# deepqmc/deepqmc

Measured on NVIDIA H100. Metric: walker.local-energies/sec, higher is better.
Workload: dtype f32

## Files before the change

deepqmc_b200/csrc/engine.cu:

```cuda
#include <algorithm>
#include <array>
#include <cstdio>
#include <cstdlib>
#include <cstring>
#include <limits>
#include <map>
#include <mutex>
#include <optional>
#include <string>
#include <type_traits>
#include <vector>

#include "dqmc_b200.h"
#include "kernels_mcmc.cuh"
#include "kernels_slater.cuh"
#include "kernels_trunk.cuh"
#include "kernels_gnn.cuh"
#include "kernels_bwd.cuh"
#include "attn_mma.cuh"
#if !defined(DQMC_NO_TCGEN05)
#include "gemm_wgmma.cuh"
#include "fused_tc.cuh"
#include "trunk_tc.cuh"
#endif

namespace dq {

struct ParamEntry {
  std::string name;
  int64_t offset;
  int rows, cols;
};

static inline size_t align_up(size_t x, size_t a = 256) { return (x + a - 1) / a * a; }

template <class W>
static double last_above(W w, double lo, double eps) {
  double hi = lo > 0.0 ? 2 * lo : 1.0;
  while (w(hi) >= eps) { lo = hi; hi *= 2; }
  for (;;) {
    const double mid = lo + 0.5 * (hi - lo);
    if (mid <= lo || mid >= hi) break;
    (w(mid) >= eps ? lo : hi) = mid;
  }
  return lo;
}

template <class T>
static double ecp_cutoff_rc2(const T* nl, int L, int Tn, bool on) {
  const double inf = std::numeric_limits<double>::infinity(), eps = std::ldexp(1.0, -100);
  if (!on) return inf;
  for (int l = 0; l < L; ++l)
    for (int t = 0; t < Tn; ++t)
      if ((double)nl[(l * 2 + 1) * Tn + t] != 0.0 && !((double)nl[(l * 2) * Tn + t] > 0.0)) return inf;
  auto w = [&](double d2) {
    double s = 0.0;
    for (int l = 0; l < L; ++l)
      for (int t = 0; t < Tn; ++t)
        s += (2 * l + 1) * std::fabs((double)nl[(l * 2 + 1) * Tn + t]) * std::exp(-(double)nl[(l * 2) * Tn + t] * d2);
    return s;
  };
  if (w(0.0) < eps) return -inf;
  return last_above(w, 0.0, eps);
}

template <class T>
static double ecp_force_cutoff_rc2(const T* nl, int L, int Tn, bool on) {
  const double rc2 = ecp_cutoff_rc2(nl, L, Tn, on), eps = std::ldexp(1.0, -100);
  if (rc2 == std::numeric_limits<double>::infinity()) return rc2;
  double peak = 0.0;
  for (int l = 0; l < L; ++l)
    for (int t = 0; t < Tn; ++t)
      if ((double)nl[(l * 2 + 1) * Tn + t] != 0.0) peak = std::max(peak, 0.5 / (double)nl[(l * 2) * Tn + t]);
  auto wd = [&](double d2) {
    double s = 0.0;
    for (int l = 0; l < L; ++l)
      for (int t = 0; t < Tn; ++t) {
        const double a = (double)nl[(l * 2) * Tn + t];
        s += (2 * l + 1) * 2 * a * std::fabs((double)nl[(l * 2 + 1) * Tn + t]) * std::sqrt(d2) * std::exp(-a * d2);
      }
    return s;
  };
  return std::max(rc2, wd(peak) >= eps ? last_above(wd, peak, eps) : peak);
}

struct Switches {
  bool tc_trunk = true;
  bool tc_f16 = true;
  std::optional<bool> attn_fl_mma;
  std::optional<int> attn_tb, attn_nt;
  bool attn_generic = false;
  bool no_fuse_tanh = false;
  bool slater_generic = false;
  bool slater_fwd1 = false;
  bool ecp_cutoff = true;
  bool ecp_env_table = true;
  bool ecp_emb_table = true;
  int nsms = 0;
  bool trunk_phases = false;
};

inline Switches read_switches() {
  auto env = [](const char* name) { return std::getenv(name); };
  auto num = [&](const char* name) { const char* ev = env(name); return ev ? std::optional<int>(std::atoi(ev)) : std::nullopt; };
  Switches s;
  s.tc_trunk = num("DQMC_TC_TRUNK").value_or(1) != 0;
  s.tc_f16 = num("DQMC_TC_F16").value_or(1) != 0;
  if (auto v = num("DQMC_ATTN_FL_MMA")) s.attn_fl_mma = *v != 0;
  s.attn_tb = num("DQMC_ATTN_TB");
  s.attn_nt = num("DQMC_ATTN_NT");
  s.attn_generic = env("DQMC_ATTN_GENERIC");
  s.no_fuse_tanh = env("DQMC_NO_FUSE_TANH");
  s.slater_generic = env("DQMC_SLATER_GENERIC");
  s.slater_fwd1 = env("DQMC_SLATER_FWD1");
  s.ecp_cutoff = num("DQMC_ECP_CUTOFF").value_or(1) != 0;
  s.ecp_env_table = !env("DQMC_ECP_ENV_TABLE_OFF");
  s.ecp_emb_table = !env("DQMC_ECP_EMB_TABLE_OFF");
  s.nsms = num("DQMC_NSMS").value_or(0);
  s.trunk_phases = num("DQMC_TRUNK_PHASES").value_or(0) != 0;
  return s;
}

struct EngineBase {
  dqmc_config cfg;
  int device = 0;
  std::string err;
  int64_t launches = 0;
  int64_t ecp_forwards = 0;
  std::vector<ParamEntry> entries;
  int64_t total = 0;
  bool dry = false;
  bool plan_only = false;
  mutable const char* dry_hwm = nullptr;
  void note_hwm(const void* q) const { if (dry && (const char*)q > dry_hwm) dry_hwm = (const char*)q; }
  mutable std::vector<unsigned char*> emu_guards;
  bool prof = false;
  double prof_flops = 0;
  int64_t prof_n = 0;
  double prof_cls_flops[3] = {0, 0, 0};
  int64_t prof_cls_n[3] = {0, 0, 0};
  std::vector<int> prof_cls;
#ifndef DQMC_EMU
  std::vector<cudaEvent_t> prof_ev;
  void prof_note(cudaEvent_t e0, cudaEvent_t e1, double flops, int cls) {
    prof_ev.push_back(e0); prof_ev.push_back(e1);
    prof_cls.push_back(cls);
    prof_flops += flops; prof_cls_flops[cls] += flops;
    ++prof_n; ++prof_cls_n[cls];
  }
#endif
  virtual ~EngineBase() {}
  virtual int set_params(const double* host, int64_t n, cudaStream_t st) = 0;
  virtual int64_t ws_bytes(int B, int mode) = 0;
  virtual int64_t ws_bytes_min(int B, int mode) = 0;
  virtual int debug_plan(int B, int mode, int64_t wsb, int64_t* planned, int64_t* carved) = 0;
  virtual int stats_pack(const void* E, const void* stats, int B, double* out, cudaStream_t st) = 0;
  virtual int debug_mlp_block(int layer, const void* O, const void* X, void* Out, int rows, cudaStream_t st) = 0;
  virtual int debug_trunk(const void* X0, void* Out, int rows, cudaStream_t st) = 0;
  virtual int debug_attention(int layer, const void* QKV, void* O, int rows, int S, int32_t* kernel, cudaStream_t st) = 0;
  virtual int debug_mlp(int layer, int S, const void* O, const void* X, void* Out, void* scratch, int rows, int32_t* path,
                        cudaStream_t st) = 0;
  virtual int debug_trunk_phases(uint64_t* out, int n) = 0;
  virtual int debug_slater(const void* r, const void* R, const void* BF, int rows, int S, void* dsign, void* dlog, void* dgrad,
                           void* dlap, int32_t* kernel, cudaStream_t st) = 0;
  virtual int debug_det_sum(const void* r, const void* R, const void* dsign, const void* dlog, const void* dgrad,
                            const void* dlap, int B, int S, void* sign, void* logp, void* grad, void* stats,
                            cudaStream_t st) = 0;
  virtual int forward(const void* r, const void* R, int Rb, int B, void* sign, void* logp, void* ws, int64_t wsb,
                      cudaStream_t st) = 0;
  virtual int local_energy(const void* r, const void* R, int Rb, int B, uint64_t seed, const void* twist, void* E,
                           void* stats, void* sign, void* logp, void* grad, void* ws, int64_t wsb,
                           cudaStream_t st) = 0;
  virtual int langevin(void* r, void* sign, void* logp, void* force, int32_t* age, void* tau, const void* R, int Rb, int B,
                       int n_sub, double target, int max_age, uint64_t seed, uint64_t step0, uint64_t woff, const void* nn,
                       const void* nu, void* stats, void* ws, int64_t wsb, cudaStream_t st) = 0;
  virtual int vjp_params(const void* r, const void* R, int Rb, int B, const void* weights, void* sign, void* logp,
                         void* grad_params, void* ws, int64_t wsb, cudaStream_t st) = 0;
  virtual int spin(const void* r, const void* R, int Rb, int B, const void* sign, const void* logp, int down_idx, void* s2,
                   void* ratio, void* ws, int64_t wsb, cudaStream_t st) = 0;
  virtual int grad_positions(const void* r, const void* R, int Rb, int B, void* sign, void* logp, void* grad_r, void* grad_R,
                             void* ws, int64_t wsb, cudaStream_t st) = 0;
  virtual int force_terms(const void* r, const void* R, int Rb, int B, const void* grad_r, void* bare, void* zvq, void* Q,
                          cudaStream_t st) = 0;
  virtual int ecp_force(const void* r, const void* R, int Rb, int B, uint64_t seed, const void* twist, void* bare, void* nl,
                        void* ws, int64_t wsb, cudaStream_t st) = 0;
  virtual int orbitals(const void* r, const void* R, int Rb, int B, void* out, void* ws, int64_t wsb, cudaStream_t st) = 0;
  virtual int set_ph(int n_tab, int n_grid, double r_max, const double* tables, const int32_t* tab_of_nuc) = 0;
  virtual int debug_gemm(const char* wname, const char* bname, const void* A, const void* Res, void* C, int Mr, int S,
                         int sliced, int backend, cudaStream_t st) = 0;
  virtual int mcmc(void* r, void* sign, void* logp, int32_t* age, void* tau, const void* R, int Rb, int B, int n_sub,
// ... 397 lines not shown
      std::vector<int> nuc;
      for (int m = 0; m < M; ++m) {
        bool any = false;
        for (int l = 0; l < L; ++l)
          for (int ab = 0; ab < 2; ++ab)
            for (int t = 0; t < Tn; ++t) {
              double v = cfg.ecp_nl[m][l][ab][t];
              np[(((size_t)m * L + l) * 2 + ab) * Tn + t] = (T)v;
              any = any || v != 0.0;
            }
        if (any) nuc.push_back(m);
      }
      J = (int)nuc.size();
      if (J > 0) {
        DQ_CHECK(cudaMalloc((void**)&d_nl_params, sizeof(T) * np.size()));
        DQ_CHECK(cudaMemcpy(d_nl_params, np.data(), sizeof(T) * np.size(), cudaMemcpyHostToDevice));
        DQ_CHECK(cudaMalloc((void**)&d_nl_nuc, sizeof(int) * J));
        DQ_CHECK(cudaMemcpy(d_nl_nuc, nuc.data(), sizeof(int) * J, cudaMemcpyHostToDevice));
        std::vector<double> rc2(J), rc2f(J);
        for (int j = 0; j < J; ++j) {
          rc2[j] = ecp_cutoff_rc2(np.data() + (size_t)nuc[j] * L * 2 * Tn, L, Tn, sw.ecp_cutoff);
          rc2f[j] = ecp_force_cutoff_rc2(np.data() + (size_t)nuc[j] * L * 2 * Tn, L, Tn, sw.ecp_cutoff);
        }
        DQ_CHECK(cudaMalloc((void**)&d_nl_rc2, sizeof(double) * J));
        DQ_CHECK(cudaMemcpy(d_nl_rc2, rc2.data(), sizeof(double) * J, cudaMemcpyHostToDevice));
        DQ_CHECK(cudaMalloc((void**)&d_nl_rc2f, sizeof(double) * J));
        DQ_CHECK(cudaMemcpy(d_nl_rc2f, rc2f.data(), sizeof(double) * J, cudaMemcpyHostToDevice));
      }
    }
#ifndef DQMC_EMU
    {
      int v = 0;
      DQ_CHECK(cudaDeviceGetAttribute(&v, cudaDevAttrMultiProcessorCount, device));
      if (v > 0) n_sms = v;
    }
#endif
    if (sw.nsms >= 1) n_sms = sw.nsms;
    const bool psif = cfg.kind == DQMC_PSIFORMER || trans;
    attn_f32 = psif && !trans && std::is_same<T, float>::value && dh % 16 == 0 && !sw.attn_generic;
    if (sw.attn_tb && *sw.attn_tb >= 1 && *sw.attn_tb <= T3) attn_tb = *sw.attn_tb;
    else attn_tb = attn_f32 ? attn_f32_pick_tb(N, dh, T3, 32 * 1024) : attn_pick_tb<T>(N, dh, T3, 100 * 1024, Mn);
    size_t s_attn = !psif ? 0 : attn_f32 ? attn_f32_smem_bytes(N, dh, attn_tb) : attn_smem_bytes<T>(N, dh, attn_tb, Mn);
    if (!sw.attn_nt) attn_fl_threads = s_attn > 110 * 1024 ? 512 : (s_attn > 56 * 1024 ? 256 : 128);
    else if (*sw.attn_nt >= 32 && *sw.attn_nt <= 1024 && *sw.attn_nt % 32 == 0) attn_fl_threads = *sw.attn_nt;
    attn_fl_mma = attn_f32 && N <= 32 && dh % 16 == 0 && sw.attn_fl_mma.value_or(N >= 20);
    if (attn_fl_mma && !sw.attn_tb) {
      attn_tb = attn_f32_pick_tb(N, dh, T3, 110 * 1024);
      s_attn = attn_f32_smem_bytes(N, dh, attn_tb);
    }
    attn_gen_mma = psif && !attn_f32 && std::is_same<T, float>::value && dh % 16 == 0 &&
                   sw.attn_fl_mma.value_or(N >= 20 && !sw.attn_generic);
    if (attn_gen_mma) {
      if (!sw.attn_tb) attn_tb = attn_pick_tb<T>(N, dh, T3, 110 * 1024, Mn, 4);
      s_attn = attn_smem_bytes<T>(N, dh, attn_tb, Mn, 4);
    }
    size_t s_sl = slater_smem_bytes<T>(N);
    max_smem = s_attn > s_sl ? s_attn : s_sl;
    if (max_smem > 227 * 1024) { err = "system too large for the shared-memory tiling (N)"; return 2; }
    if (attn_f32) {
      if (launch_attn_f32(nullptr, nullptr, 0, 0, 0, 0.f, 0, (int)s_attn, nullptr, true)) return 1;
    } else if (psif) {
      DQ_CHECK(raise_dyn_smem(attn_fl_kernel<T>, (int)s_attn));
      if constexpr (std::is_same<T, float>::value) DQ_CHECK(raise_dyn_smem((attn_fl_kernel<T, true>), (int)s_attn));
    }
    DQ_CHECK(raise_dyn_smem(slater_kernel<T>, (int)s_sl));
    slater_fwd2_ok = N <= 32 && slater_fwd2_smem_bytes<T>(N, M, K) <= 110 * 1024 && !sw.slater_generic && !sw.slater_fwd1;
    if (slater_fwd2_ok) {
      DQ_CHECK(raise_dyn_smem(slater_fwd2_kernel<T, 14>, (int)slater_fwd2_smem_bytes<T>(N, M, K)));
      DQ_CHECK(raise_dyn_smem(slater_fwd2_kernel<T, 16>, (int)slater_fwd2_smem_bytes<T>(N, M, K)));
      DQ_CHECK(raise_dyn_smem(slater_fwd2_kernel<T, 28>, (int)slater_fwd2_smem_bytes<T>(N, M, K)));
      DQ_CHECK(raise_dyn_smem(slater_fwd2_kernel<T, 30>, (int)slater_fwd2_smem_bytes<T>(N, M, K)));
      DQ_CHECK(raise_dyn_smem(slater_fwd2_kernel<T, 32>, (int)slater_fwd2_smem_bytes<T>(N, M, K)));
    }
    attn_mma_ok = psif && std::is_same<T, float>::value && dh == 64 && N + Mn <= 48 && d % 4 == 0 && !sw.attn_generic;
    embed_fwd_ok = psif && d % 4 == 0 && embed_fwd_smem_bytes<T>(M, d) <= 200 * 1024;
    if (embed_fwd_ok)
      DQ_CHECK(raise_dyn_smem(embed_fwd_kernel<T>, (int)embed_fwd_smem_bytes<T>(M, d)));
    if (cfg.gemm_backend == DQMC_GEMM_TCGEN05) {
#if !defined(DQMC_NO_TCGEN05)
      if (!std::is_same<T, float>::value) { err = "DQMC_GEMM_TCGEN05 needs dtype DQMC_F32"; return 2; }
      if (d % 32 != 0) { err = "DQMC_GEMM_TCGEN05 needs embedding_dim % 32 == 0"; return 2; }
      DQ_CHECK(raise_dyn_smem(tc::gemm3x_kernel<false>, tc::SmemLayout::total()));
      DQ_CHECK(raise_dyn_smem(tc::gemm3x_kernel<true>, tc::SmemLayout::total()));
      DQ_CHECK(raise_dyn_smem(tc::mlp_block_f16_kernel<128>, tc::MlpSmem::total()));
      DQ_CHECK(raise_dyn_smem(tc::mlp_block_f16_kernel<256>, tc::MlpSmem::total()));
      DQ_CHECK(raise_dyn_smem(tc::trunk_f16_kernel<1>, tc::TrSmem::total()));
      DQ_CHECK(raise_dyn_smem(tc::trunk_f16_kernel<2>, tc::TrSmem::total()));
      DQ_CHECK(raise_dyn_smem(tc::trunk_f16_kernel<4>, tc::TrSmem::total()));
      DQ_CHECK(raise_dyn_smem(tc::trunk_f16_kernel<8>, tc::TrSmem::total()));
      DQ_CHECK(raise_dyn_smem(tc::trunk_f16_kernel<16>, tc::TrSmem::total()));
      DQ_CHECK(raise_dyn_smem(tc::trunk_f16_kernel<32>, tc::TrSmem::total()));
      if (psif && !trans && d == 256 && H == 4 && N <= 32 && cfg.n_layers <= tc::kTrMaxLayers) {
        DQ_CHECK(cudaMalloc((void**)&d_trunk_maps, sizeof(CUtensorMap) * 8 * cfg.n_layers));
        DQ_CHECK(cudaMalloc((void**)&d_trunk_scratch, (size_t)n_sms * tc::kTrScratchPerCta));
        if (sw.trunk_phases) {
          DQ_CHECK(cudaMalloc((void**)&d_trunk_phase, sizeof(unsigned long long) * tc::kPhases));
          DQ_CHECK(cudaMemset(d_trunk_phase, 0, sizeof(unsigned long long) * tc::kPhases));
        }
      }
#else
      err = "this build has no tensor-core backend"; return 2;
#endif
    }
    return 0;
  }
  ~Engine() override {
    if (plan_only) return;
    cudaFree(d_params); cudaFree(d_params_t); cudaFree(d_stage); cudaFree(d_znuc); cudaFree(d_zval); cudaFree(d_ecp_mask);
    if (d_ecp_loc) cudaFree(d_ecp_loc);
    if (d_nl_params) cudaFree(d_nl_params);
    if (d_nl_nuc) cudaFree(d_nl_nuc);
    if (d_nl_rc2) cudaFree(d_nl_rc2);
    if (d_nl_rc2f) cudaFree(d_nl_rc2f);
    if (d_ph_tabs) cudaFree(d_ph_tabs);
    if (d_ph_nuc) cudaFree(d_ph_nuc);
#if !defined(DQMC_NO_TCGEN05)
    for (auto& kv : tcw) {
      if (kv.second.hi) cudaFree(kv.second.hi);
      if (kv.second.lo) cudaFree(kv.second.lo);
      if (kv.second.h16) cudaFree(kv.second.h16);
    }
    if (d_trunk_maps) cudaFree(d_trunk_maps);
    if (d_trunk_scratch) cudaFree(d_trunk_scratch);
    if (d_trunk_phase) cudaFree(d_trunk_phase);
#endif
  }
  const T* P(const std::string& n) const { return d_params + off(n); }

  int set_ph(int n_tab, int n_grid, double r_max, const double* tables, const int32_t* tab_of_nuc) override {
    if (J > 0 || cfg.ecp_loc_terms > 0) { err = "pseudo-Hamiltonian and Gaussian-type ECP are mutually exclusive"; return 2; }
    if (n_tab < 1 || n_grid < 2 || !(r_max > 0) || !tables || !tab_of_nuc) { err = "bad pseudo-Hamiltonian tables"; return 2; }
    for (int m = 0; m < M; ++m)
      if (tab_of_nuc[m] >= n_tab) { err = "pseudo-Hamiltonian table index out of range"; return 2; }
    std::vector<T> h((size_t)n_tab * 2 * n_grid);
    for (size_t i = 0; i < h.size(); ++i) h[i] = (T)tables[i];
    if (d_ph_tabs) cudaFree(d_ph_tabs);
    if (d_ph_nuc) cudaFree(d_ph_nuc);
    DQ_CHECK(cudaMalloc((void**)&d_ph_tabs, sizeof(T) * h.size()));
    DQ_CHECK(cudaMemcpy(d_ph_tabs, h.data(), sizeof(T) * h.size(), cudaMemcpyHostToDevice));
    DQ_CHECK(cudaMalloc((void**)&d_ph_nuc, sizeof(int) * M));
    DQ_CHECK(cudaMemcpy(d_ph_nuc, tab_of_nuc, sizeof(int) * M, cudaMemcpyHostToDevice));
    ph_G = n_grid; ph_rmax = r_max; ph_on = true;
    return 0;
  }
  PhArgs<T> ph_args(const T* QA) const {
    PhArgs<T> a;
    a.QA = QA; a.tabs = d_ph_tabs; a.tab_of_nuc = d_ph_nuc; a.G = ph_G; a.rmax = (T)ph_rmax;
    return a;
  }

  int set_params(const double* host, int64_t n, cudaStream_t st) override {
    if (n != total) { err = "parameter count mismatch"; return 2; }
    DQ_CHECK(cudaMemcpyAsync(d_stage, host, sizeof(double) * n, cudaMemcpyHostToDevice, st));
    DQ_LAUNCH(convert_kernel<T>, dim3((unsigned)((n + 255) / 256)), dim3(256), 0, st, (const double*)d_stage, d_params, n);
    for (auto& e : entries)
      if (e.rows >= 1 && e.cols >= 1)
        DQ_LAUNCH(transpose_kernel<T>, dim3((e.rows * e.cols + 255) / 256), dim3(256), 0, st, (const T*)(d_params + e.offset),
                  e.rows, e.cols, d_params_t + e.offset);
#if !defined(DQMC_NO_TCGEN05)
    if (use_tc()) {
      std::map<std::string, double> wmax;
      auto group = [](const std::string& n) {
        const size_t k = n.size();
        return (k > 3 && (n.compare(k - 3, 3, ".up") == 0 || n.compare(k - 3, 3, ".dn") == 0)) ? n.substr(0, k - 3) : n;
      };
      for (auto& e : entries) {
// ... 215 lines not shown
    if (B < 1) B = 1;
    const int S = T3 + 2;
    switch (mode) {
      case DQMC_MODE_VJP: return vjp_chunk_bytes(1);
      case DQMC_MODE_GRAD_POS: return has_pos_pass() ? vjp_chunk_bytes(1, true) : 0;
      case DQMC_MODE_MCMC: return sweep_bytes(B, false, 1);
      case DQMC_MODE_LANGEVIN: return sweep_bytes(B, true, 1);
      case DQMC_MODE_LOCAL_ENERGY: return std::max<int64_t>(chunk_bytes(1, S), J > 0 ? ecp_bytes(1, 1) : 0);
      case DQMC_MODE_ECP_FORCE: return J > 0 && has_nl_force() ? ecp_force_bytes(1, 1) : 0;
      case DQMC_MODE_SPIN: {
        const int64_t P = (int64_t)cfg.n_up * cfg.n_down;
        return P ? spin_bytes(1, P, 1) : 0;
      }
      default: return chunk_bytes(1, 1);
    }
  }
  int debug_plan(int B, int mode, int64_t wsb, int64_t* planned, int64_t* carved) override {
    const int64_t pl = ws_bytes(B, mode);
    if (planned) *planned = pl;
    if (wsb <= 0) wsb = pl;
    DryPass dp(this);
    void* ws = plan_base();
    int rc = 0;
    switch (mode) {
      case DQMC_MODE_FORWARD: rc = forward(nullptr, nullptr, 0, B, nullptr, nullptr, ws, wsb, nullptr); break;
      case DQMC_MODE_LOCAL_ENERGY:
        rc = local_energy(nullptr, nullptr, 0, B, 0, nullptr, nullptr, nullptr, nullptr, nullptr, nullptr, ws, wsb, nullptr);
        break;
      case DQMC_MODE_VJP: rc = vjp_params(nullptr, nullptr, 0, B, nullptr, nullptr, nullptr, nullptr, ws, wsb, nullptr); break;
      case DQMC_MODE_MCMC:
        rc = mcmc(nullptr, nullptr, nullptr, nullptr, nullptr, nullptr, 0, B, 1, 0.5, -1, 0, 0, 0, nullptr, nullptr, nullptr, ws, wsb,
                  nullptr, 0.0, nullptr, nullptr);
        break;
      case DQMC_MODE_LANGEVIN:
        rc = langevin(nullptr, nullptr, nullptr, nullptr, nullptr, nullptr, nullptr, 0, B, 1, 0.5, -1, 0, 0, 0, nullptr, nullptr,
                      nullptr, ws, wsb, nullptr);
        break;
      case DQMC_MODE_SPIN: rc = spin(nullptr, nullptr, 0, B, nullptr, nullptr, -1, nullptr, nullptr, ws, wsb, nullptr); break;
      case DQMC_MODE_GRAD_POS:
        rc = grad_positions(nullptr, nullptr, 0, B, nullptr, nullptr, nullptr, nullptr, ws, wsb, nullptr);
        break;
      case DQMC_MODE_ECP_FORCE:
        rc = ecp_force(nullptr, nullptr, 0, B, 0, nullptr, nullptr, has_nl_force() ? ws : nullptr, ws, wsb, nullptr);
        break;
      default: err = "unknown mode"; rc = 2;
    }
    if (carved) *carved = dp.bytes();
    return rc;
  }

  bool can_fuse_act(int S) const {
    if (!use_tc() || sw.no_fuse_tanh) return false;
    if (S == 1) return true;
    return S <= 128 && (128 / S) * S >= 112;
  }
  bool gemm_on_tc(const char* w0, const char* w1, int lda, int ldc, int Kc, const T* bias1) const {
#if !defined(DQMC_NO_TCGEN05)
    return use_tc() && !bias1 && Kc % 32 == 0 && lda % 4 == 0 && ldc % 4 == 0 && tcw.count(w0) && (!w1 || tcw.count(w1));
#else
    return false;
#endif
  }
  int gemm(const T* A, int lda, const char* w0, const char* w1, int zsplit, int ldw, const T* bias, const T* Res,
           int ldr, T* C, int ldc, int Mr, int Nc, int Kc, int S, int sliced, int Nel, cudaStream_t st, int act = 0,
           const T* bias1 = nullptr) {
    if (dry) return 0;
    const T* W0 = P(w0);
    const T* W1 = w1 ? P(w1) : nullptr;
#if !defined(DQMC_NO_TCGEN05)
    if constexpr (std::is_same<T, float>::value) {
      if (gemm_on_tc(w0, w1, lda, ldc, Kc, bias1)) {
        const TcWeight& t0 = tcw.at(w0);
        const TcWeight& t1 = w1 ? tcw.at(w1) : t0;
        tc::Params p;
        p.A = A; p.lda = lda; p.bias = bias; p.Res = Res; p.ldr = ldr; p.C = C; p.ldc = ldc; p.M = Mr; p.N = Nc;
        p.K = Kc; p.S = S; p.sliced = sliced; p.Nel = Nel; p.z_split = zsplit; p.err_flag = nullptr;
        p.act = act;
        p.rpt = (act && S > 1) ? (128 / S) * S : tc::kBM;
        p.a_scale = 1.f; p.unscale = 1.f;
        const bool f16 = S == 1 && sw.tc_f16 && Kc % 64 == 0 && t0.f16 && t1.f16 && t0.wscale == t1.wscale;
        if (f16) { p.a_scale = kActScale; p.unscale = 1.f / (kActScale * t0.wscale); }
        const int MT = (Mr + p.rpt - 1) / p.rpt, NT = (Nc + tc::kBN - 1) / tc::kBN;
        const int n_tiles = (sliced ? Nel : 1) * MT * NT;
#ifndef DQMC_EMU
        cudaEvent_t e0 = nullptr, e1 = nullptr;
        if (prof) { cudaEventCreate(&e0); cudaEventCreate(&e1); cudaEventRecord(e0, st); }
#endif
        if (f16)
          DQ_LAUNCH(tc::gemm3x_kernel<true>, dim3(n_tiles), dim3(tc::kThreads), tc::SmemLayout::total(), st, t0.m16h, t0.m16l,
                    t1.m16h, t1.m16l, p);
        else
          DQ_LAUNCH(tc::gemm3x_kernel<false>, dim3(n_tiles), dim3(tc::kThreads), tc::SmemLayout::total(), st, t0.mh, t0.ml,
                    t1.mh, t1.ml, p);
#ifndef DQMC_EMU
        if (prof) {
          cudaEventRecord(e1, st);
          prof_note(e0, e1, 2.0 * (double)Mr * (sliced ? Nel : 1) * (double)Nc * (double)Kc, 0);
        }
#endif
        return 0;
      }
    }
#endif
    if (act) { err = "internal: fused activation requested on the CUDA-core GEMM"; return 5; }
    GemmArgs<T> g;
    g.A = A; g.lda = lda; g.W0 = W0; g.W1 = W1; g.z_split = zsplit; g.ldw = ldw; g.bias = bias; g.Res = Res;
    g.ldr = ldr; g.C = C; g.ldc = ldc; g.M = Mr; g.N = Nc; g.K = Kc; g.S = S; g.sliced = sliced; g.Nel = Nel;
    g.bias1 = bias1;
    constexpr int BM = 64, BN = 64, BK = 16, TM = 4, TN = 4;
    dim3 grid((Nc + BN - 1) / BN, (Mr + BM - 1) / BM, sliced ? Nel : 1);
#ifndef DQMC_EMU
    cudaEvent_t e0 = nullptr, e1 = nullptr;
    if (prof) { cudaEventCreate(&e0); cudaEventCreate(&e1); cudaEventRecord(e0, st); }
#endif
    DQ_LAUNCH((gemm_kernel<T, BM, BN, BK, TM, TN>), grid, dim3(256), 0, st, g);
#ifndef DQMC_EMU
    if (prof) {
      cudaEventRecord(e1, st);
      prof_note(e0, e1, 2.0 * (double)Mr * (sliced ? Nel : 1) * (double)Nc * (double)Kc, 0);
    }
#endif
    return 0;
  }

  bool can_fuse_mlp(int S, const std::string& pfx) const {
#if !defined(DQMC_NO_TCGEN05)
    if (S != 1 || !use_tc() || !sw.tc_f16 || (d != 128 && d != 256)) return false;
    for (const char* n : {"wo", "w1", "w2"}) {
      auto it = tcw.find(pfx + n);
      if (it == tcw.end() || !it->second.f16_all) return false;
    }
    return true;
#else
    return false;
#endif
  }
  int mlp_block(const std::string& pfx, const T* O, const T* X, T* Out, int rows, cudaStream_t st) {
    if (dry) return 0;
#if !defined(DQMC_NO_TCGEN05)
    if constexpr (std::is_same<T, float>::value) {
      const TcWeight& wo = tcw.at(pfx + "wo");
      const TcWeight& w1 = tcw.at(pfx + "w1");
      const TcWeight& w2 = tcw.at(pfx + "w2");
      tc::MlpParams p;
      p.O = O; p.ldo = d; p.X = X; p.ldx = d; p.Out = Out; p.ldout = d; p.b1 = P(pfx + "b1"); p.b2 = P(pfx + "b2");
      p.M = rows; p.d = d; p.a_scale = kActScale;
      p.us0 = 1.f / (kActScale * wo.wscale); p.us1 = 1.f / (kActScale * w1.wscale); p.us2 = 1.f / (kActScale * w2.wscale);
      p.err_flag = nullptr;
      const int MT = (rows + 127) / 128;
      const int grid = MT < n_sms ? MT : n_sms;
#ifndef DQMC_EMU
      cudaEvent_t e0 = nullptr, e1 = nullptr;
      if (prof) { cudaEventCreate(&e0); cudaEventCreate(&e1); cudaEventRecord(e0, st); }
#endif
      if (d == 256)
        DQ_LAUNCH(tc::mlp_block_f16_kernel<256>, dim3(grid), dim3(tc::kMlpThreads), tc::MlpSmem::total(), st, wo.m16h_all,
                  wo.m16l_all, w1.m16h_all, w1.m16l_all, w2.m16h_all, w2.m16l_all, p);
      else
        DQ_LAUNCH(tc::mlp_block_f16_kernel<128>, dim3(grid), dim3(tc::kMlpThreads), tc::MlpSmem::total(), st, wo.m16h_all,
                  wo.m16l_all, w1.m16h_all, w1.m16l_all, w2.m16h_all, w2.m16l_all, p);
#ifndef DQMC_EMU
      if (prof) {
        cudaEventRecord(e1, st);
        prof_note(e0, e1, 3 * 2.0 * (double)rows * (double)d * (double)d, 1);
      }
#endif
      return 0;
    }
#endif
    err = "internal: fused MLP block without the tensor-core backend";
    return 5;
  }

  int debug_mlp_block(int layer, const void* O, const void* X, void* Out, int rows, cudaStream_t st) override {
    const std::string pfx = "L" + std::to_string(layer) + ".";
    if (!can_fuse_mlp(1, pfx)) { err = "fused MLP block not available for this configuration"; return 2; }
// ... 1785 lines not shown
```

deepqmc_b200/csrc/gemm_wgmma.cuh:

```cuda
#pragma once
#include <cstdint>

#include "tc_ptx.cuh"

namespace dq {
namespace tc {

constexpr int kBM = 128;
constexpr int kBN = 128;
constexpr int kBK = 32;
constexpr int kThreads = 256;

struct Params {
  const float* A; int lda;
  const float* bias;
  const float* Res; int ldr;
  float* C; int ldc;
  int M, N, K;
  int S;
  int sliced, Nel, z_split;
  int act;
  int rpt;
  int* err_flag;
  float a_scale;
// ... 141 lines not shown
  }
  __syncthreads();

  constexpr int P = SmemLayout::kPitch;
  float* st = (float*)smem;
  {
    const int lane = tid & 31;
    const int fr = 64 * wg + 16 * ((tid >> 5) & 3) + (lane >> 2), fc = 2 * (lane & 3);
    const float us = F16 ? p.unscale : 1.f;
#pragma unroll
    for (int j = 0; j < kBN / 8; ++j)
#pragma unroll
      for (int h = 0; h < 2; ++h)
        *(float2*)(st + (fr + 8 * h) * P + 8 * j + fc) = make_float2(acc[4 * j + 2 * h] * us, acc[4 * j + 2 * h + 1] * us);
  }
  __syncthreads();
  const int S = p.S;
  const int rows_here = (p.M - mt * RPT) < RPT ? (p.M - mt * RPT) : RPT;
  const int col0 = nt * kBN;
  if (p.act) {
    if (S == 1) {
      for (int idx = tid; idx < rows_here * kBN; idx += kThreads) {
        const int r = idx / kBN, c = idx % kBN;
        const float b = (p.bias && col0 + c < p.N) ? __ldg(p.bias + col0 + c) : 0.f;
        st[r * P + c] = tanh_fwd(st[r * P + c] + b);
      }
    } else {
      const int ngrp = rows_here / S;
      for (int idx = tid; idx < ngrp * kBN; idx += kThreads) {
        const int g = idx / kBN, c = idx % kBN;
        float* zp = st + g * S * P + c;
        const float b = (p.bias && col0 + c < p.N) ? __ldg(p.bias + col0 + c) : 0.f;
        const float y = tanhf(zp[0] + b);
        const float y1 = 1.f - y * y, y2 = -2.f * y * y1;
        float s0 = 0.f, s1 = 0.f;
        int t = 1;
        for (; t + 1 <= S - 2; t += 2) {
          const float a0 = zp[t * P], a1 = zp[(t + 1) * P];
          s0 += a0 * a0; s1 += a1 * a1;
        }
        for (; t <= S - 2; ++t) {
          const float a = zp[t * P];
          s0 += a * a;
        }
        zp[0] = y;
        for (int u = 1; u < S - 1; ++u) zp[u * P] *= y1;
        zp[(S - 1) * P] = y1 * zp[(S - 1) * P] + y2 * (s0 + s1);
      }
    }
    __syncthreads();
  }
  const float* __restrict__ Resp = p.Res;
  float* __restrict__ Cp = p.C;
  const bool vec_ok = (p.N % 4) == 0 && (p.ldc % 4) == 0 && (!Resp || (p.ldr % 4) == 0);
  if (vec_ok) {
    for (int idx = tid; idx < rows_here * (kBN / 4); idx += kThreads) {
      const int r = idx / (kBN / 4), c = 4 * (idx % (kBN / 4)), col = col0 + c;
      if (col >= p.N) continue;
      const size_t pr = phys_row(p, mt * RPT + r, z);
      float4 o = *(const float4*)(st + r * P + c);
      if (Resp) {
        const float4 q = __ldg((const float4*)(Resp + pr * p.ldr + col));
        o.x += q.x; o.y += q.y; o.z += q.z; o.w += q.w;
      }
      if (p.bias && !p.act && pr % S == 0) {
        const float4 q = __ldg((const float4*)(p.bias + col));
        o.x += q.x; o.y += q.y; o.z += q.z; o.w += q.w;
      }
      *(float4*)(Cp + pr * p.ldc + col) = o;
    }
  } else {
    for (int idx = tid; idx < rows_here * kBN; idx += kThreads) {
      const int r = idx / kBN, c = idx % kBN, col = col0 + c;
      if (col >= p.N) continue;
      const size_t pr = phys_row(p, mt * RPT + r, z);
      float o = st[r * P + c];
      if (Resp) o += Resp[pr * p.ldr + col];
      if (p.bias && !p.act && pr % S == 0) o += p.bias[col];
      Cp[pr * p.ldc + col] = o;
    }
  }
}

inline int make_weight_map(CUtensorMap* map, const float* wt, int Nrows, int K, int BN) {
  return make_kmajor_map(map, wt, 4, Nrows, K, kBK, BN);
}

}
}
```

Baseline: 888.0.

## Add persistent warp-specialized row GEMM with producer, MMA, and epilogue warpgroups

Adds a persistent wgmma GEMM kernel, launched with one CTA per SM, that splits work across four warpgroups. One warpgroup loads and splits activations into hi/lo parts while TMA fetches weights into a two-stage mbarrier ring. Two warpgroups issue the wgmma ops and one runs the bias/tanh/residual epilogue. It is used by default when the K dimension spans 4-8 blocks, so loads, MMA and epilogue of successive tiles can overlap and per-tile launch overhead goes away. The cost is extra barrier complexity, and with only one CTA per SM, small grids may lose parallelism.

New measurement: 907.0 (median of 6 runs). 1.02x the previous value.

```diff
diff --git a/deepqmc_b200/csrc/engine.cu b/deepqmc_b200/csrc/engine.cu
--- a/deepqmc_b200/csrc/engine.cu
+++ b/deepqmc_b200/csrc/engine.cu
@@ -87,6 +87,7 @@
 struct Switches {
   bool tc_trunk = true;
   bool tc_f16 = true;
+  bool row_gemm_ws = true;
   std::optional<bool> attn_fl_mma;
   std::optional<int> attn_tb, attn_nt;
   bool attn_generic = false;
@@ -106,6 +107,7 @@
   Switches s;
   s.tc_trunk = num("DQMC_TC_TRUNK").value_or(1) != 0;
   s.tc_f16 = num("DQMC_TC_F16").value_or(1) != 0;
+  s.row_gemm_ws = num("DQMC_ROW_GEMM_WS").value_or(1) != 0;
   if (auto v = num("DQMC_ATTN_FL_MMA")) s.attn_fl_mma = *v != 0;
   s.attn_tb = num("DQMC_ATTN_TB");
   s.attn_nt = num("DQMC_ATTN_NT");
@@ -669,6 +671,8 @@
       if (d % 32 != 0) { err = "DQMC_GEMM_TCGEN05 needs embedding_dim % 32 == 0"; return 2; }
       DQ_CHECK(raise_dyn_smem(tc::gemm3x_kernel<false>, tc::SmemLayout::total()));
       DQ_CHECK(raise_dyn_smem(tc::gemm3x_kernel<true>, tc::SmemLayout::total()));
+      DQ_CHECK(raise_dyn_smem(tc::rowgemm_ws_kernel<false>, tc::WsSmem::total()));
+      DQ_CHECK(raise_dyn_smem(tc::rowgemm_ws_kernel<true>, tc::WsSmem::total()));
       DQ_CHECK(raise_dyn_smem(tc::mlp_block_f16_kernel<128>, tc::MlpSmem::total()));
       DQ_CHECK(raise_dyn_smem(tc::mlp_block_f16_kernel<256>, tc::MlpSmem::total()));
       DQ_CHECK(raise_dyn_smem(tc::trunk_f16_kernel<1>, tc::TrSmem::total()));
@@ -1050,16 +1054,27 @@
         if (f16) { p.a_scale = kActScale; p.unscale = 1.f / (kActScale * t0.wscale); }
         const int MT = (Mr + p.rpt - 1) / p.rpt, NT = (Nc + tc::kBN - 1) / tc::kBN;
         const int n_tiles = (sliced ? Nel : 1) * MT * NT;
+        const int grid = n_tiles < n_sms ? n_tiles : n_sms;
+        const int kblocks = Kc / (tc::kBK * (f16 ? 2 : 1));
+        const bool ws = sw.row_gemm_ws && kblocks >= 4 && kblocks <= 8;
 #ifndef DQMC_EMU
         cudaEvent_t e0 = nullptr, e1 = nullptr;
         if (prof) { cudaEventCreate(&e0); cudaEventCreate(&e1); cudaEventRecord(e0, st); }
 #endif
-        if (f16)
+        if (ws) {
+          if (f16)
+            DQ_LAUNCH(tc::rowgemm_ws_kernel<true>, dim3(grid), dim3(tc::kWsThreads), tc::WsSmem::total(), st, t0.m16h, t0.m16l,
+                      t1.m16h, t1.m16l, p);
+          else
+            DQ_LAUNCH(tc::rowgemm_ws_kernel<false>, dim3(grid), dim3(tc::kWsThreads), tc::WsSmem::total(), st, t0.mh, t0.ml,
+                      t1.mh, t1.ml, p);
+        } else if (f16) {
           DQ_LAUNCH(tc::gemm3x_kernel<true>, dim3(n_tiles), dim3(tc::kThreads), tc::SmemLayout::total(), st, t0.m16h, t0.m16l,
                     t1.m16h, t1.m16l, p);
-        else
+        } else {
           DQ_LAUNCH(tc::gemm3x_kernel<false>, dim3(n_tiles), dim3(tc::kThreads), tc::SmemLayout::total(), st, t0.mh, t0.ml,
                     t1.mh, t1.ml, p);
+        }
 #ifndef DQMC_EMU
         if (prof) {
           cudaEventRecord(e1, st);
diff --git a/deepqmc_b200/csrc/gemm_wgmma.cuh b/deepqmc_b200/csrc/gemm_wgmma.cuh
--- a/deepqmc_b200/csrc/gemm_wgmma.cuh
+++ b/deepqmc_b200/csrc/gemm_wgmma.cuh
@@ -247,6 +247,247 @@
   }
 }
 
+constexpr int kWsThreads = 512;
+
+struct WsSmem {
+  static constexpr int kStages = 2;
+  static constexpr int kEpi = kStages * SmemLayout::kStageBytes;
+  static constexpr int kBars = kEpi + kBM * SmemLayout::kPitch * 4;
+  static constexpr int total() { return kBars + 64; }
+};
+static_assert(WsSmem::total() <= 227 * 1024, "stages + epilogue tile must fit the shared memory of an SM");
+
+template <bool F16>
+__global__ void __launch_bounds__(kWsThreads, 1)
+rowgemm_ws_kernel(const __grid_constant__ CUtensorMap map_hi0, const __grid_constant__ CUtensorMap map_lo0,
+                  const __grid_constant__ CUtensorMap map_hi1, const __grid_constant__ CUtensorMap map_lo1, Params p) {
+  DQMC_TC_SMEM(smem);
+  if ((smem_u32(smem) & 1023u) != 0u) tc_trap();
+  constexpr int kSt = WsSmem::kStages;
+  uint64_t* full = (uint64_t*)(smem + WsSmem::kBars);
+  uint64_t* empty = full + kSt;
+  uint64_t* epi_full = empty + kSt;
+  uint64_t* epi_empty = epi_full + 1;
+  float* st = (float*)(smem + WsSmem::kEpi);
+  constexpr int P = SmemLayout::kPitch;
+  const int tid = threadIdx.x, wg = tid >> 7, wtid = tid & 127;
+  const int RPT = p.rpt;
+  const int MT = (p.M + RPT - 1) / RPT, NT = (p.N + kBN - 1) / kBN;
+  const int n_tiles = (p.sliced ? p.Nel : 1) * MT * NT;
+  constexpr int kSub = F16 ? 2 : 1;
+  const int KS = p.K / (kBK * kSub);
+
+  if (tid == 0) {
+    for (int s = 0; s < kSt; ++s) {
+      mbar_init(&full[s], 1 + 128);
+      mbar_init(&empty[s], 8);
+    }
+    mbar_init(epi_full, 256);
+    mbar_init(epi_empty, 128);
+    fence_barrier_init();
+    tma_prefetch_desc(&map_hi0);
+    tma_prefetch_desc(&map_lo0);
+    if (p.sliced) {
+      tma_prefetch_desc(&map_hi1);
+      tma_prefetch_desc(&map_lo1);
+    }
+  }
+  __syncthreads();
+
+  if (wg == 0) {
+    constexpr int kChunks = F16 ? 16 : 8;
+    constexpr int kRows = kBM * kChunks / 128;
+    constexpr int kRowStep = 128 / kChunks;
+    const int chunk = wtid % kChunks, r0 = wtid / kChunks;
+    int it = 0;
+    for (int tile = blockIdx.x; tile < n_tiles; tile += gridDim.x) {
+      const int nt = tile % NT, mt = (tile / NT) % MT, z = tile / (NT * MT);
+      const bool second = p.sliced && z >= p.z_split;
+      const CUtensorMap* mh = second ? &map_hi1 : &map_hi0;
+      const CUtensorMap* ml = second ? &map_lo1 : &map_lo0;
+      const float* rowp[kRows];
+#pragma unroll
+      for (int i = 0; i < kRows; ++i) {
+        const int lrow = r0 + kRowStep * i, m = mt * RPT + lrow;
+        rowp[i] = (lrow < RPT && m < p.M) ? p.A + phys_row(p, m, z) * p.lda + chunk * 4 : nullptr;
+      }
+      for (int ks = 0; ks < KS; ++ks, ++it) {
+        const int s = it % kSt;
+        float4 av[kRows];
+#pragma unroll
+        for (int i = 0; i < kRows; ++i)
+          av[i] = rowp[i] ? __ldg((const float4*)(rowp[i] + ks * kBK * kSub)) : make_float4(0.f, 0.f, 0.f, 0.f);
+        mbar_wait(&empty[s], ((it / kSt) & 1) ^ 1, p.err_flag);
+        if (wtid == 0) {
+          mbar_expect_tx(&full[s], 2u * kBN * 128u);
+          tma_load_2d(mh, &full[s], smem + SmemLayout::w_hi(s), ks * kBK * kSub, nt * kBN);
+          tma_load_2d(ml, &full[s], smem + SmemLayout::w_lo(s), ks * kBK * kSub, nt * kBN);
+        }
+        unsigned char* ah = smem + SmemLayout::a_hi(s);
+        unsigned char* al = smem + SmemLayout::a_lo(s);
+#pragma unroll
+        for (int i = 0; i < kRows; ++i) {
+          const int trow = r0 + kRowStep * i;
+          if constexpr (F16) {
+            const float sc = p.a_scale;
+            const float x0 = av[i].x * sc, x1 = av[i].y * sc, x2 = av[i].z * sc, x3 = av[i].w * sc;
+            const uint32_t h01 = pack_half2_rn(x0, x1), h23 = pack_half2_rn(x2, x3);
+            const uint32_t l01 = pack_half2_rn(x0 - half_bits_to_float(h01 & 0xFFFFu), x1 - half_bits_to_float(h01 >> 16));
+            const uint32_t l23 = pack_half2_rn(x2 - half_bits_to_float(h23 & 0xFFFFu), x3 - half_bits_to_float(h23 >> 16));
+            const int c16 = chunk >> 1;
+            const int off = trow * 128 + ((c16 ^ (trow & 7)) << 4) + (chunk & 1) * 8;
+            *(uint2*)(ah + off) = make_uint2(h01, h23);
+            *(uint2*)(al + off) = make_uint2(l01, l23);
+          } else {
+            float4 v = av[i], h, l;
+            h.x = tf32_rna(v.x); l.x = tf32_rna(v.x - h.x);
+            h.y = tf32_rna(v.y); l.y = tf32_rna(v.y - h.y);
+            h.z = tf32_rna(v.z); l.z = tf32_rna(v.z - h.z);
+            h.w = tf32_rna(v.w); l.w = tf32_rna(v.w - h.w);
+            const int off = trow * 128 + ((chunk ^ (trow & 7)) << 4);
+            *(float4*)(ah + off) = h;
+            *(float4*)(al + off) = l;
+          }
+        }
+        fence_proxy_async();
+        mbar_arrive(&full[s]);
+      }
+    }
+  } else if (wg <= 2) {
+    const int mw = wg - 1;
+    const float us = F16 ? p.unscale : 1.f;
+    float acc[kBN / 2];
+#pragma unroll
+    for (int i = 0; i < kBN / 2; ++i) acc[i] = 0.f;
+    int it = 0, tn = 0;
+    for (int tile = blockIdx.x; tile < n_tiles; tile += gridDim.x, ++tn) {
+      for (int ks = 0; ks < KS; ++ks, ++it) {
+        const int s = it % kSt;
+        mbar_wait(&full[s], (it / kSt) & 1, p.err_flag);
+        const uint32_t ah = smem_u32(smem + SmemLayout::a_hi(s)) + mw * 8192, al = smem_u32(smem + SmemLayout::a_lo(s)) + mw * 8192;
+        const uint32_t wh = smem_u32(smem + SmemLayout::w_hi(s)), wl = smem_u32(smem + SmemLayout::w_lo(s));
+        wgmma_fence();
+#pragma unroll
+        for (int k = 0; k < 4; ++k) {
+          const uint32_t ko = k * 32;
+          const int first = (ks | k) ? 1 : 0;
+          if constexpr (F16) {
+            wgmma_f16_n128(acc, make_desc(al + ko), make_desc(wh + ko), first);
+            wgmma_f16_n128(acc, make_desc(ah + ko), make_desc(wh + ko), 1);
+            wgmma_f16_n128(acc, make_desc(ah + ko), make_desc(wl + ko), 1);
+          } else {
+            wgmma_tf32_n128(acc, make_desc(al + ko), make_desc(wh + ko), first);
+            wgmma_tf32_n128(acc, make_desc(ah + ko), make_desc(wh + ko), 1);
+            wgmma_tf32_n128(acc, make_desc(ah + ko), make_desc(wl + ko), 1);
+          }
+        }
+        wgmma_commit();
+        if (ks > 0) {
+          wgmma_wait1();
+          if ((tid & 31) == 0) mbar_arrive(&empty[(it - 1) % kSt]);
+        }
+      }
+      wgmma_wait0();
+      fence_acc(acc);
+      if ((tid & 31) == 0) mbar_arrive(&empty[(it - 1) % kSt]);
+      mbar_wait(epi_empty, (tn & 1) ^ 1, p.err_flag);
+      const int lane = tid & 31;
+      const int fr = 64 * mw + 16 * ((tid >> 5) & 3) + (lane >> 2), fc = 2 * (lane & 3);
+#pragma unroll
+      for (int j = 0; j < kBN / 8; ++j)
+#pragma unroll
+        for (int h = 0; h < 2; ++h)
+          *(float2*)(st + (fr + 8 * h) * P + 8 * j + fc) = make_float2(acc[4 * j + 2 * h] * us, acc[4 * j + 2 * h + 1] * us);
+      mbar_arrive(epi_full);
+    }
+  } else {
+    int tn = 0;
+    for (int tile = blockIdx.x; tile < n_tiles; tile += gridDim.x, ++tn) {
+      const int nt = tile % NT, mt = (tile / NT) % MT, z = tile / (NT * MT);
+      mbar_wait(epi_full, tn & 1, p.err_flag);
+      const int S = p.S;
+      const int rows_here = (p.M - mt * RPT) < RPT ? (p.M - mt * RPT) : RPT;
+      const int col0 = nt * kBN;
+      if (p.act) {
+        if (S == 1) {
+          for (int idx = wtid; idx < rows_here * kBN; idx += 128) {
+            const int r = idx / kBN, c = idx % kBN;
+            const float b = (p.bias && col0 + c < p.N) ? __ldg(p.bias + col0 + c) : 0.f;
+            st[r * P + c] = tanh_fwd(st[r * P + c] + b);
+          }
+        } else {
+          const int ngrp = rows_here / S;
+          for (int idx = wtid; idx < ngrp * kBN; idx += 128) {
+            const int g = idx / kBN, c = idx % kBN;
+            float* zp = st + g * S * P + c;
+            const float b = (p.bias && col0 + c < p.N) ? __ldg(p.bias + col0 + c) : 0.f;
+            const float y = tanhf(zp[0] + b);
+            const float y1 = 1.f - y * y, y2 = -2.f * y * y1;
+            float s0 = 0.f, s1 = 0.f;
+            int t = 1;
+            for (; t + 1 <= S - 2; t += 2) {
+              const float a0 = zp[t * P], a1 = zp[(t + 1) * P];
+              s0 += a0 * a0; s1 += a1 * a1;
+            }
+            for (; t <= S - 2; ++t) {
+              const float a = zp[t * P];
+              s0 += a * a;
+            }
+            zp[0] = y;
+            for (int u = 1; u < S - 1; ++u) zp[u * P] *= y1;
+            zp[(S - 1) * P] = y1 * zp[(S - 1) * P] + y2 * (s0 + s1);
+          }
+        }
+        wg_sync(wg);
+      }
+      const float* __restrict__ Resp = p.Res;
+      float* __restrict__ Cp = p.C;
+      const bool vec_ok = (p.N % 4) == 0 && (p.ldc % 4) == 0 && (!Resp || (p.ldr % 4) == 0);
+      if (vec_ok) {
+        constexpr int kRes = 8;
+        const int n4 = rows_here * (kBN / 4);
+        for (int i0 = wtid; i0 < n4; i0 += 128 * kRes) {
+          float4 q[kRes];
+#pragma unroll
+          for (int u = 0; u < kRes; ++u) {
+            const int idx = i0 + 128 * u, col = col0 + 4 * (idx % (kBN / 4));
+            q[u] = (Resp && idx < n4 && col < p.N)
+                       ? __ldg((const float4*)(Resp + phys_row(p, mt * RPT + idx / (kBN / 4), z) * p.ldr + col))
+                       : make_float4(0.f, 0.f, 0.f, 0.f);
+          }
+#pragma unroll
+          for (int u = 0; u < kRes; ++u) {
+            const int idx = i0 + 128 * u;
+            const int r = idx / (kBN / 4), c = 4 * (idx % (kBN / 4)), col = col0 + c;
+            if (idx >= n4 || col >= p.N) continue;
+            const size_t pr = phys_row(p, mt * RPT + r, z);
+            float4 o = *(const float4*)(st + r * P + c);
+            if (Resp) {
+              o.x += q[u].x; o.y += q[u].y; o.z += q[u].z; o.w += q[u].w;
+            }
+            if (p.bias && !p.act && pr % S == 0) {
+              const float4 q = __ldg((const float4*)(p.bias + col));
+              o.x += q.x; o.y += q.y; o.z += q.z; o.w += q.w;
+            }
+            *(float4*)(Cp + pr * p.ldc + col) = o;
+          }
+        }
+      } else {
+        for (int idx = wtid; idx < rows_here * kBN; idx += 128) {
+          const int r = idx / kBN, c = idx % kBN, col = col0 + c;
+          if (col >= p.N) continue;
+          const size_t pr = phys_row(p, mt * RPT + r, z);
+          float o = st[r * P + c];
+          if (Resp) o += Resp[pr * p.ldr + col];
+          if (p.bias && !p.act && pr % S == 0) o += p.bias[col];
+          Cp[pr * p.ldc + col] = o;
+        }
+      }
+      mbar_arrive(epi_empty);
+    }
+  }
+}
+
 inline int make_weight_map(CUtensorMap* map, const float* wt, int Nrows, int K, int BN) {
   return make_kmajor_map(map, wt, 4, Nrows, K, kBK, BN);
 }
```
